# ZwwWayne/mmMOT

Measured on AMD Instinct MI355X. Metric: frame-pairs/sec (fusion+affinity fwd) at N_det=64; affinity L∞ vs CPU ref, higher is better.
Workload: dtype f16x3

## Files before the change

### include/mmmot_hip.h

```cpp
#ifndef MMMOT_HIP_H
#define MMMOT_HIP_H

#include <stddef.h>
#include <stdint.h>

#ifdef __cplusplus
extern "C" {
#endif

#define MMMOT_OK 0
#define MMMOT_EINVAL (-1)

#define MMMOT_ACT_NONE 0
#define MMMOT_ACT_RELU 1
#define MMMOT_ACT_SIGMOID 2

#define MMMOT_A_PLAIN 0
#define MMMOT_A_NORM_RELU 1
#define MMMOT_A_PAIR 2

#define MMMOT_PAIR_MULTIPLY 0
#define MMMOT_PAIR_MINUS_ABS 1
#define MMMOT_PAIR_MINUS 2

// ... 7 lines not shown

#define MMMOT_FUSION_A 0
#define MMMOT_FUSION_B 1
#define MMMOT_FUSION_C 2

int mmmot_abi_version(void);
int mmmot_device_info(int device, int* cu_count, char* arch, int arch_len);

int mmmot_conv3x3_bn_relu(const float* in, const float* wp, const float* bias,
                          float* out, int L, int H, int W, int Cin, int Cout,
                          int first, int pool, void* stream);

int mmmot_conv3x3_bn_relu_hl16_patch(const void* in, const void* wp, const float* bias, void* out,
                                     int L, int H, int W, int Cin, int Cout, int pool, const float* oscale,
                                     void* stream);
int mmmot_conv1_fused_hl16(const float* crops, const void* w1, const float* bias1, float oscale1,
                           const void* w2, const float* bias2, const float* oscale2, void* out, int L, int H, int W,
                           void* stream);
int mmmot_conv1_fused_u8(const unsigned char* crops_u8, float mean0, float mean1, float mean2, float std0, float std1,
                         float std2, const void* w1, const float* bias1, float oscale1, const void* w2,
                         const float* bias2, const float* oscale2, void* out, int L, int H, int W, int q8, void* stream);
int mmmot_conv3x3_bn_relu_hq8(const void* in, const void* wp, const float* bias, void* out,
                              int L, int H, int W, int Cin, int Cout, int pool, const float* oscale, void* stream);
int mmmot_conv1_fused_hq8(const float* crops, const void* w1, const float* bias1, float oscale1,
                          const void* w2, const float* bias2, const float* oscale2, void* out, int L, int H, int W,
                          void* stream);
int mmmot_hq8_pack(const float* x, void* y, long n, void* stream);
int mmmot_hq8_unpack(const void* x, float* y, long n, void* stream);
int mmmot_trunk_range_read(unsigned int* out4, int reset);
int mmmot_trunk_range_bind(unsigned int* counters4);
// ... 278 lines not shown
```

### mmmot_amd/_lib.py

```python
import ctypes
import os
import subprocess
import threading

_HERE = os.path.dirname(os.path.abspath(__file__))
CSRC = os.path.join(_HERE, 'csrc')
LIB_PATH = os.environ.get('MMMOT_LIB_PATH', os.path.join(_HERE, 'libmmmot_hip.so'))
SOURCES = ['conv3x3.hip', 'hl16_format.hip', 'conv3x3_hl16_patch.hip', 'gemm_rows.hip', 'gemm_wide.hip',
           'gemm_ares.hip', 'gemm_wres.hip', 'gemm_wreg.hip', 'pn_mlp64.hip', 'gram.hip', 'points_gather.hip', 'crop_resize.hip', 'crop_augment.hip','small_kernels.hip', 'backward.hip', 'train.hip', 'train_vgg.hip', 'gemm_tn_f16.hip',
           'assign.hip', 'assign_chain.hip', 'track_ids.hip', 'clear_mot.hip', 'align_points.hip', 'labels.hip', 'adam_step.hip', 'dropout.hip']
HIPCC = os.environ.get('HIPCC', '/opt/rocm/bin/hipcc')
HIPFLAGS = ['--offload-arch=gfx950', '-O3', '-std=c++17', '-fPIC']

_lock = threading.Lock()
_lib = None

c_f = ctypes.c_void_p
c_i = ctypes.c_int


class GemmArgs(ctypes.Structure):
    _fields_ = [
        ('X', c_f), ('ldx', c_i),
        ('W', c_f),
# ... 47 lines not shown
    'mmmot_abi_version': [],
    'mmmot_device_info': [c_i, ctypes.POINTER(c_i), ctypes.c_char_p, c_i],
    'mmmot_conv3x3_bn_relu': [c_f, c_f, c_f, c_f, c_i, c_i, c_i, c_i, c_i, c_i, c_i, c_f],
    'mmmot_gemm_rows': [ctypes.POINTER(GemmArgs), c_f],
    'mmmot_set_gemm_rows_variant': [c_i],
    'mmmot_gemm_ares': [ctypes.POINTER(GemmAresArgs), c_f],
    'mmmot_set_gemm_ares_variant': [c_i],
    'mmmot_gram_rows': [c_f, c_i, c_i, c_f, c_f, c_i, c_f, c_f, c_f, c_i, c_f, c_f, c_f],
    'mmmot_set_gram128_variant': [c_i],
    'mmmot_gn_finalize_gram': [c_f, c_f, c_f, c_f, c_f, c_i, c_i, c_f, c_f, c_i, c_f, c_f, ctypes.c_float, c_f, c_f, c_f, c_f],
    'mmmot_gn_finalize_gram_dbias': [c_f, c_f, c_f, c_f, c_f, c_i, c_f, c_f, c_i, c_f, c_f, c_i, c_i, c_f, c_f, ctypes.c_float,
                                     c_f, c_f, c_f, c_f],
    'mmmot_gn_finalize': [c_f, c_f, c_f, c_f, c_f, c_i, c_i, c_i, c_i, c_f, c_f, ctypes.c_float, c_f, c_f, c_f],
    'mmmot_segment_mean': [c_f, c_i, c_i, c_f, c_f, c_f, c_f, c_f, c_i, c_f, c_f, c_i, c_i, c_f, c_i, c_i, c_f],
    'mmmot_conv3x3_bn_relu_hl16_patch': [c_f, c_f, c_f, c_f, c_i, c_i, c_i, c_i, c_i, c_i, c_f, c_f],
    'mmmot_conv1_fused_hl16': [c_f, c_f, c_f, ctypes.c_float, c_f, c_f, c_f, c_f, c_i, c_i, c_i, c_f],
    'mmmot_conv3x3_bn_relu_hq8': [c_f, c_f, c_f, c_f, c_i, c_i, c_i, c_i, c_i, c_i, c_f, c_f],
    'mmmot_conv1_fused_u8': [c_f, ctypes.c_float, ctypes.c_float, ctypes.c_float, ctypes.c_float, ctypes.c_float,
                             ctypes.c_float, c_f, c_f, ctypes.c_float, c_f, c_f, c_f, c_f, c_i, c_i, c_i, c_i, c_f],
    'mmmot_u8_normalize': [c_f, c_i, c_i, c_f, c_f, c_f],
    'mmmot_conv1_fused_hq8': [c_f, c_f, c_f, ctypes.c_float, c_f, c_f, c_f, c_f, c_i, c_i, c_i, c_f],
    'mmmot_conv3x3_first_hl16': [c_f, c_f, c_f, c_f, c_i, c_i, c_i, c_i, c_f],
    'mmmot_set_patch_grid_limit': [c_i],
    'mmmot_set_patch_min_block': [c_i],
    'mmmot_trunk_range_read': [ctypes.POINTER(ctypes.c_uint), c_i],
    'mmmot_trunk_range_bind': [c_f],
    'mmmot_hl16_pack': [c_f, c_f, ctypes.c_long, c_f],
    'mmmot_hl16_unpack': [c_f, c_f, ctypes.c_long, c_f],
    'mmmot_hl16_pack_pow2': [c_f, c_f, ctypes.c_long, c_f, c_i, c_f],
    'mmmot_pow2_oscale': [c_f, c_i, c_f, c_i, c_f, c_i, c_f],
# ... 136 lines not shown
```

### mmmot_amd/csrc/conv3x3_hl16_patch.hip

```cpp
#include <atomic>
#include <type_traits>

#include "common.h"

#include "patch_common.h"

template <int BN, int BS, bool POOL, bool FUSE1 = false, bool Q8 = false, bool RAW = false PT_TIMED_TPARAM>
__global__ __launch_bounds__(512) void conv3x3_hl16_patch_kernel(
    const u32x4* __restrict__ in, const u32x4* __restrict__ wp, const float* __restrict__ bias,
    u32x4* __restrict__ out, int L, int H, int W, int Cin, int Cout, int nby, int nbx, int nblk, int ntm, int ntn,
    const float* __restrict__ oscv, Fuse1Args fz, unsigned int* __restrict__ rng) {
#include "patch_setup.inc"
  for (int item = blockIdx.x >> 3; item < clen; item += gridDim.x >> 3) {
#include "patch_loaders.inc"
#include "patch_fragments.inc"
#include "patch_prologue.inc"
#include "patch_kloop.inc"
#include "patch_epilogue.inc"
  }
}


static thread_local unsigned int* g_range_bound = nullptr;
extern "C" int mmmot_trunk_range_bind(unsigned int* counters4) {
  if (counters4 && (((uintptr_t)counters4) & 3u)) return MMMOT_EINVAL;
  g_range_bound = counters4;
// ... 44 lines not shown
  if (H <= 4 && W <= 4 && g_patch_min_block.load() != 8) return 4;
  return 8;
}

static bool pt_use_bn64(int L, int H, int W, int Cout) {
  if (Cout % 128 != 0) return true;
  const int n_cu = pt_num_cu();
  if (n_cu <= 0) return false;
  const int bs = pt_block_edge(H, W), nb = 256 / (bs * bs);
  const long nblk = (long)L * ((H + bs - 1) / bs) * ((W + bs - 1) / bs);
  const long i128 = ((nblk + nb - 1) / nb) * (Cout / 128), i64 = 2 * i128;
  auto eff = [&](long items) { return (double)items / (double)(((items + n_cu - 1) / n_cu) * n_cu); };
  return 0.85 * eff(i64) > eff(i128);
}

template <int BN, int BS, bool POOL, bool FUSE1 = false, bool Q8 = false, bool RAW = false PT_TIMED_TPARAM>
static int launch_patch_e(const void* in, const void* wp, const float* bias, void* out, int L, int H, int W, int Cin,
                        int Cout, const float* oscale, hipStream_t s, Fuse1Args fz = Fuse1Args{nullptr, nullptr, nullptr, 1.f, nullptr, {0.f, 0.f, 0.f}, {1.f, 1.f, 1.f}}) {
  const int nby = (H + BS - 1) / BS, nbx = (W + BS - 1) / BS;
  const int nblk = L * nby * nbx;
  constexpr int NB = PatchGeom<BS>::NB;
  const int ntm = (nblk + NB - 1) / NB;
  const int ntn = Cout / BN;
  const int n_cu = pt_num_cu();
  if (n_cu <= 0) return MMMOT_EINVAL;
  const int nitems = ntm * ntn;
  int grid = (n_cu / 8) * 8;
  const int glimit = g_patch_grid_limit.load();
  if (glimit > 0 && grid > glimit) grid = glimit;
  if (grid > ((nitems + 7) / 8) * 8) grid = ((nitems + 7) / 8) * 8;
  unsigned int* rng = pt_range_block();
  if (!rng) return MMMOT_EINVAL;
  hipLaunchKernelGGL((conv3x3_hl16_patch_kernel<BN, BS, POOL, FUSE1, Q8, RAW PT_TIMED_TARG(TIMED)>), dim3(grid), dim3(512), 0, s,
                     (const u32x4*)in, (const u32x4*)wp, bias, (u32x4*)out, L, H, W, Cin, Cout, nby, nbx, nblk, ntm, ntn,
                     oscale, fz, rng);
  return mm_check(hipGetLastError());
}

template <int BN, int BS, bool POOL>
static int launch_patch(const void* in, const void* wp, const float* bias, void* out, int L, int H, int W, int Cin,
                        int Cout, const float* oscale, hipStream_t s) {
#ifdef MMMOT_DEBUG
  if constexpr (BN == 128 && BS == 16)
    if (g_patch_timed) return launch_patch_e<BN, BS, POOL, false, false, false, true>(in, wp, bias, out, L, H, W, Cin, Cout, oscale, s);
#endif
  return launch_patch_e<BN, BS, POOL>(in, wp, bias, out, L, H, W, Cin, Cout, oscale, s);
}

template <int BN, int BS>
static int launch_patch_p(int pool, const void* in, const void* wp, const float* bias, void* out, int L, int H, int W,
                          int Cin, int Cout, const float* oscale, hipStream_t s) {
  return pool ? launch_patch<BN, BS, true>(in, wp, bias, out, L, H, W, Cin, Cout, oscale, s)
              : launch_patch<BN, BS, false>(in, wp, bias, out, L, H, W, Cin, Cout, oscale, s);
}

extern "C" int mmmot_conv3x3_bn_relu_hl16_patch(const void* in, const void* wp, const float* bias, void* out, int L,
                                                int H, int W, int Cin, int Cout, int pool, const float* oscale,
                                                void* stream) {
  hipStream_t s = (hipStream_t)stream;
  if (!in || !wp || !bias || !out || !oscale || L <= 0 || H <= 0 || W <= 0) return MMMOT_EINVAL;
  if (Cin % 32 != 0 || Cout % 64 != 0) return MMMOT_EINVAL;
  if (!mm_al16(in) || !mm_al16(wp) || !mm_al16(out)) return MMMOT_EINVAL;
  if ((long)L * H * W * (Cin / 4) >= (1L << 31) - 64) return MMMOT_EINVAL;
  const int bs = pt_block_edge(H, W);
  if (!pt_use_bn64(L, H, W, Cout))
    return bs == 16 ? launch_patch_p<128, 16>(pool, in, wp, bias, out, L, H, W, Cin, Cout, oscale, s)
           : bs == 8 ? launch_patch_p<128, 8>(pool, in, wp, bias, out, L, H, W, Cin, Cout, oscale, s)
                     : launch_patch_p<128, 4>(pool, in, wp, bias, out, L, H, W, Cin, Cout, oscale, s);
  return bs == 16 ? launch_patch_p<64, 16>(pool, in, wp, bias, out, L, H, W, Cin, Cout, oscale, s)
         : bs == 8 ? launch_patch_p<64, 8>(pool, in, wp, bias, out, L, H, W, Cin, Cout, oscale, s)
                   : launch_patch_p<64, 4>(pool, in, wp, bias, out, L, H, W, Cin, Cout, oscale, s);
}

extern "C" int mmmot_conv3x3_raw_hl16(const void* in, const void* wp, const float* bias, float* out, int L, int H, int W,
                                      int Cin, int Cout, const float* oscale, void* stream) {
  hipStream_t s = (hipStream_t)stream;
  if (!in || !wp || !bias || !out || !oscale || L <= 0 || H <= 0 || W <= 0) return MMMOT_EINVAL;
  if (Cin % 32 != 0 || Cout % 64 != 0) return MMMOT_EINVAL;
  if (!mm_al16(in) || !mm_al16(wp) || !mm_al16(out)) return MMMOT_EINVAL;
  if ((long)L * H * W * (Cin / 4) >= (1L << 31) - 64) return MMMOT_EINVAL;
  const int bs = pt_block_edge(H, W);
#define PT_RAW(BNV, BSV) launch_patch_e<BNV, BSV, false, false, false, true>(in, wp, bias, out, L, H, W, Cin, Cout, oscale, s)
  if (!pt_use_bn64(L, H, W, Cout)) return bs == 16 ? PT_RAW(128, 16) : bs == 8 ? PT_RAW(128, 8) : PT_RAW(128, 4);
  return bs == 16 ? PT_RAW(64, 16) : bs == 8 ? PT_RAW(64, 8) : PT_RAW(64, 4);
#undef PT_RAW
}

extern "C" int mmmot_conv1_fused_hl16(const float* crops, const void* w1, const float* bias1, float oscale1,
                                      const void* w2, const float* bias2, const float* oscale2, void* out, int L, int H,
                                      int W, void* stream) {
  hipStream_t s = (hipStream_t)stream;
  if (!crops || !w1 || !bias1 || !w2 || !bias2 || !oscale2 || !out || L <= 0 || H <= 0 || W <= 0) return MMMOT_EINVAL;
  if ((H & 1) || (W & 1) || !mm_al16(w1) || !mm_al16(w2) || !mm_al16(out)) return MMMOT_EINVAL;
  Fuse1Args fz{crops, (const u32x4*)w1, bias1, oscale1, nullptr, {0.f, 0.f, 0.f}, {1.f, 1.f, 1.f}};
#ifdef MMMOT_DEBUG
  if (g_patch_timed) return launch_patch_e<64, 16, true, true, false, false, true>(nullptr, w2, bias2, out, L, H, W, 64, 64, oscale2, s, fz);
#endif
  return launch_patch_e<64, 16, true, true>(nullptr, w2, bias2, out, L, H, W, 64, 64, oscale2, s, fz);
}

extern "C" int mmmot_conv1_fused_u8(const unsigned char* crops_u8, float mean0, float mean1, float mean2, float std0,
                                    float std1, float std2, const void* w1, const float* bias1, float oscale1,
                                    const void* w2, const float* bias2, const float* oscale2, void* out, int L, int H,
                                    int W, int q8, void* stream) {
  hipStream_t s = (hipStream_t)stream;
  if (!crops_u8 || !w1 || !bias1 || !w2 || !bias2 || !oscale2 || !out || L <= 0 || H <= 0 || W <= 0) return MMMOT_EINVAL;
  if ((H & 1) || (W & 1) || !mm_al16(w1) || !mm_al16(w2) || !mm_al16(out)) return MMMOT_EINVAL;
  if (!(std0 != 0.f) || !(std1 != 0.f) || !(std2 != 0.f)) return MMMOT_EINVAL;
  Fuse1Args fz{nullptr, (const u32x4*)w1, bias1, oscale1, crops_u8, {mean0, mean1, mean2}, {std0, std1, std2}};
  if (q8) return launch_patch_e<64, 16, true, true, true>(nullptr, w2, bias2, out, L, H, W, 64, 64, oscale2, s, fz);
  return launch_patch_e<64, 16, true, true>(nullptr, w2, bias2, out, L, H, W, 64, 64, oscale2, s, fz);
}

template <int BN, int BS>
static int launch_q8_p(int pool, const void* in, const void* wp, const float* bias, void* out, int L, int H, int W,
                       int Cin, int Cout, const float* oscale, hipStream_t s) {
#ifdef MMMOT_DEBUG
  if constexpr (BN == 128 && BS == 16)
    if (!pool && g_patch_timed) return launch_patch_e<BN, BS, false, false, true, false, true>(in, wp, bias, out, L, H, W, Cin, Cout, oscale, s);
#endif
  return pool ? launch_patch_e<BN, BS, true, false, true>(in, wp, bias, out, L, H, W, Cin, Cout, oscale, s)
              : launch_patch_e<BN, BS, false, false, true>(in, wp, bias, out, L, H, W, Cin, Cout, oscale, s);
}

extern "C" int mmmot_conv3x3_bn_relu_hq8(const void* in, const void* wp, const float* bias, void* out, int L, int H,
                                         int W, int Cin, int Cout, int pool, const float* oscale, void* stream) {
  hipStream_t s = (hipStream_t)stream;
  if (!in || !wp || !bias || !out || !oscale || L <= 0 || H <= 0 || W <= 0) return MMMOT_EINVAL;
  if (Cin % 32 != 0 || Cout % 64 != 0) return MMMOT_EINVAL;
  if (!mm_al16(in) || !mm_al16(wp) || !mm_al16(out)) return MMMOT_EINVAL;
  if ((long)L * H * W * (Cin / 4) >= (1L << 31) - 64) return MMMOT_EINVAL;
  const int bs = pt_block_edge(H, W);
  if (!pt_use_bn64(L, H, W, Cout))
    return bs == 16 ? launch_q8_p<128, 16>(pool, in, wp, bias, out, L, H, W, Cin, Cout, oscale, s)
// ... 69 lines not shown
```

### mmmot_amd/csrc/patch_epilogue.inc

```
  if constexpr (FUSE1 && !OVL) {
    raw_ready = has_next;
    if (raw_ready) fetch_raw(mt_next);
  }
  constexpr int UN = BN / 8;
  constexpr int RSTEP = 512 / UN;
  const int eu = tid % UN, er0 = tid / UN;
  const f32x8 bv = *reinterpret_cast<const f32x8*>(&bias[n0 + eu * 8]);
  const f32x8 sv = *reinterpret_cast<const f32x8*>(&oscv[n0 + eu * 8]);
  constexpr int UN16 = BN / 16;
  constexpr int RSTEP16 = 512 / UN16;
  const int eu16 = tid % UN16, er16 = tid / UN16;
  float bq[16], sq[16];
  if constexpr (Q8) {
#pragma unroll
    for (int e = 0; e < 16; ++e) {
      bq[e] = bias[n0 + eu16 * 16 + e];
      sq[e] = oscv[n0 + eu16 * 16 + e];
    }
  }
  int bcrop[G::NTB], bgy0[G::NTB], bgx0[G::NTB];
#pragma unroll
  for (int k = 0; k < G::NTB; ++k) {
    const int b = mt * G::NB + k;
    const int crop = b / nbpc;
// ... 109 lines not shown
            o[6 + hf] = l8;
          }
        }
      }
    }
  } else if constexpr (POOL) {
    const int Hq = H >> 1, Wq = W >> 1;
    constexpr int NQ = RCH;
    constexpr int NIT = (NQ + RSTEP - 1) / RSTEP;
    f32x4 va[NIT], vb[NIT];
#pragma unroll
    for (int i = 0; i < NIT; ++i) {
      const int qdl = er0 + i * RSTEP;
      mm_lds_read32(mm_lds_addr(&Cs[(qdl < NQ ? qdl : 0) * CLD + eu * 8]), va[i], vb[i]);
    }
    mm_lds_wait();
    __builtin_amdgcn_sched_barrier(0);
#pragma unroll
    for (int i = 0; i < NIT; ++i) {
      const int qdl = er0 + i * RSTEP;
      const int qd = ch * NQ + qdl;
      if (qdl >= NQ) continue;
      int blk, y, x;
      pt_row_to_pixel<BS>(qd >> 3, (qd & 7) * 4, blk, y, x);
      PT_BLK_PIXEL(blk, y, x)
      if (crop >= 0 && gy < H && gx < W && (gy >> 1) < Hq && (gx >> 1) < Wq) {
        f32x8 v = {va[i][0], va[i][1], va[i][2], va[i][3], vb[i][0], vb[i][1], vb[i][2], vb[i][3]};
#pragma unroll
        for (int e = 0; e < 8; ++e) v[e] = fmaxf(fmaf(v[e], sv[e], bv[e]), 0.f);
        {
          float vg[8];
#pragma unroll
          for (int e = 0; e < 8; ++e) vg[e] = v[e];
          pt_range_guard<8>(vg, false, rng);
        }
        u32x4 hi, lo;
        pt_split8(v, hi, lo);
        const long pix = ((long)crop * Hq + (gy >> 1)) * Wq + (gx >> 1);
        u32x4* o = out + (pix * cout8 + (n0 >> 3) + eu) * 2;
        o[0] = hi;
        o[1] = lo;
      }
    }
  } else {
    constexpr int NIT = RCH / RSTEP;
    f32x4 va[NIT], vb[NIT];
#pragma unroll
    for (int i = 0; i < NIT; ++i) mm_lds_read32(mm_lds_addr(&Cs[(er0 + i * RSTEP) * CLD + eu * 8]), va[i], vb[i]);
    mm_lds_wait();
    __builtin_amdgcn_sched_barrier(0);
#pragma unroll
    for (int i = 0; i < NIT; ++i) {
      const int rl = er0 + i * RSTEP;
      const int r = ch * RCH + rl;
      int blk, y, x;
      pt_row_to_pixel<BS>(r >> 5, r & 31, blk, y, x);
// ... 53 lines not shown
```

### mmmot_amd/csrc/patch_setup.inc

```
  static_assert(!FUSE1 || (BN == 64 && BS == 16), "the fused first layer exists for 64-channel 16x16 tiles");
  static_assert(!RAW || (!POOL && !FUSE1 && !Q8), "raw fp32 output: plain unpooled f16x3 layers");
  using G = PatchGeom<BS>;
  constexpr int WN = (BN == 128) ? 2 : 1;
  constexpr int WM = 8 / WN;
  constexpr int TM = P_BM / (WM * 32);
  constexpr int TN = BN / (WN * 32);
  constexpr int B_BYTES = BN * P_ROWB;
  constexpr int NBL = BN / 64;
  constexpr int CLD = BN + 4;
  constexpr int P0_OFF = 0;
  constexpr int P1_OFF = G::BYTES;
  constexpr int RING0 = 2 * G::BYTES;
  constexpr int LOOP_BYTES = RING0 + 3 * B_BYTES;
  constexpr int RAW_OFF = LOOP_BYTES;
  constexpr int RAW_BYTES = FUSE1 ? 3 * 20 * 20 * 4 + 64 : 0;
  constexpr bool OVL = FUSE1 && !Q8;
  constexpr int SROWS = POOL ? P_BM / 4 : P_BM;
  constexpr int NCH = (FUSE1 || POOL) ? 1 : (SROWS / 2 * CLD * 4 <= G::BYTES) ? 2 : 4;
  constexpr int RCH = SROWS / NCH;
  static_assert((FUSE1 && !OVL) ? (SROWS * CLD * 4 <= LOOP_BYTES) : (RCH * CLD * 4 <= G::BYTES), "epilogue staging does not fit");
  constexpr bool STREAM = !FUSE1 && (G::NB == 1 || G::WHOLE);
  constexpr int P2_OFF = (LOOP_BYTES + RAW_BYTES + 255) / 256 * 256;
  constexpr int POFF_OFF = OVL ? P2_OFF + G::BYTES : LOOP_BYTES + RAW_BYTES;
  constexpr int W1_OFF = POFF_OFF;
  constexpr int ZOFF = POFF_OFF + (STREAM ? G::PA * 512 * 4 : 0) + (FUSE1 ? 8192 : 0);
  static_assert(ZOFF % 256 == 0, "zero page: one aligned bank row");
  constexpr int SMEM = ZOFF + (G::WHOLE ? 256 : 0);
  static_assert(SMEM <= 160 * 1024, "LDS budget");
  __shared__ __attribute__((aligned(1024))) unsigned char smem[SMEM];

  const int tid = threadIdx.x;
  const int lane = tid & 63;
  const int wave = __builtin_amdgcn_readfirstlane(tid >> 6);
  if constexpr (G::WHOLE) {
    if (tid < 16) reinterpret_cast<u32x4*>(smem + ZOFF)[tid] = u32x4{0u, 0u, 0u, 0u};
  }

  int roff[8];
  f16x8 w1h[4], w1l[4];
  if constexpr (FUSE1) {
    const int kg1 = (threadIdx.x & 63) >> 4;
    {
// ... 154 lines not shown
```

### mmmot_amd/engine.py

```python
import contextlib
import itertools
import os
import threading

import numpy as np
import torch

from .ops import (ACT_NONE, ACT_RELU, ACT_SIGMOID, A_NORM_RELU, A_PAIR, A_PLAIN, FUSION_MODES, PAIR_OPS,
                  SOFTMAX_MODES)
from .range_guard import RangeGuard
from .tape import norm_layer

POOL_INPUT = {'f32': 0, 'hl16': 1, 'hq8': 2}
EPS = 1e-5
_SERIALS = itertools.count(1)


def check_crop_side(S):
    if S < 32 or S % 2 != 0:
        raise ValueError('crop side %d is not supported: the HIP VGG trunk needs an even side >= 32; resize the crops '
                         '(mmmot_amd.crops.crop_resize_normalize)' % S)


def check_crop_layout(dets):
# ... 24 lines not shown
        self.range_events = []
        self.last_out_of_range_forward = None
        self.out_of_range_window = None
        self._busy = threading.Lock()
        self._last_stream = None
        self._head_start = None
        ql = os.environ.get('MMMOT_Q8_LAYERS', '4,5,6,7,8,9,10,11,12')
        self.q8_layers = None if ql == 'all' else set(int(v) for v in ql.split(',') if v)
        self.pn_fused = os.environ.get('MMMOT_PN_FUSED', '1') != '0'
        self.pn_gram = os.environ.get('MMMOT_PN_GRAM', '1') != '0'
        self.pn_mlp64 = os.environ.get('MMMOT_PN_MLP64', '1') != '0'
        self.two_streams = os.environ.get('MMMOT_TWO_STREAMS', '0') == '1'
        self.pn_beside_trunk = os.environ.get('MMMOT_PN_BESIDE_TRUNK', '1') != '0'
        self._side = {}
        self.sp_fused = os.environ.get('MMMOT_SP_FUSED', '1') != '0'
        self.fuse_conv1 = os.environ.get('MMMOT_FUSE_CONV1', '1') != '0'
        self.q8_min_crop = int(os.environ.get('MMMOT_Q8_MIN_CROP', '64'))
        self.mlp = 'f32' if trunk == 'f32' else 'f16x3'
        if affinity_op not in PAIR_OPS:
            raise ValueError('unknown affinity_op %r' % (affinity_op,))
        if softmax_mode not in SOFTMAX_MODES and softmax_mode != 'none':
            softmax_mode = 'none'
        self.end_mode = end_mode
        self.P = packed
        self.ops = ops
        self.fusion = fusion
        self.affinity_op = affinity_op
        self.softmax_mode = softmax_mode
        self.neg_threshold = float(neg_threshold)
        self.score_arch = score_arch
# ... 94 lines not shown
        fmt = 'raw'
        for li, cv in enumerate(vgg):
            if fuse1 and li == 0:
                continue
            lq8 = q8 and (self.q8_layers is None or li in self.q8_layers)
            want = 'hq8' if lq8 else 'hl16'
            if f16 and fmt in ('hl16', 'hq8') and fmt != want:
                n = Lt * H * W * cv['cin']
                tmp = self.buf('vgg_recode32', n)
                (ops.hq8_unpack if fmt == 'hq8' else ops.hl16_unpack)(x, tmp)
                x = self.buf('vgg_recode', n)
                (ops.hq8_pack if want == 'hq8' else ops.hl16_pack)(tmp, x)
                fmt = want
            Ho, Wo = (H // 2, W // 2) if cv['pool'] else (H, W)
            out = self.buf('vgg%d' % (li & 1), Lt * Ho * Wo, cv['cout'])
            if self.conv_events is not None:
                e0, e1 = torch.cuda.Event(enable_timing=True), torch.cuda.Event(enable_timing=True)
                e0.record()
            if fuse1 and li == 1:
                c0 = vgg[0]
                if u8:
                    from .crops import MEAN, STD
                    ops.conv1_fused_u8(x, MEAN, STD, c0['wp16'], c0['bias'], c0['oscale'], cv['wpq8'] if lq8 else cv['wp16'],
                                       cv['bias'], cv['oscale'], out, Lt, H, W, q8=lq8)
                elif lq8:
                    ops.conv1_fused_hq8(x, c0['wp16'], c0['bias'], c0['oscale'], cv['wpq8'], cv['bias'], cv['oscale'],
                                        out, Lt, H, W)
                else:
                    ops.conv1_fused_hl16(x, c0['wp16'], c0['bias'], c0['oscale'], cv['wp16'], cv['bias'],
                                         cv['oscale'], out, Lt, H, W)
# ... 1 lines not shown
            elif f16 and li == 0:
                nq8 = q8 and (self.q8_layers is None or 1 in self.q8_layers)
                if nq8:
                    tmp = self.buf('vgg_first32', Lt * H * W, cv['cout'])
                    ops.conv3x3(x, cv['wp'], cv['bias'], tmp, Lt, H, W, cv['cin'], cv['cout'], True, cv['pool'])
                    ops.hq8_pack(tmp, out)
                else:
                    ops.conv3x3_first_hl16(x, cv['wp'], cv['bias'], out, Lt, H, W, cv['cout'])
                fmt = 'hq8' if nq8 else 'hl16'
            elif lq8:
                ops.conv3x3_hq8(x, cv['wpq8'], cv['bias'], out, Lt, H, W, cv['cin'], cv['cout'], cv['pool'], cv['oscale'])
                fmt = 'hq8'
            elif not f16:
                ops.conv3x3(x, cv['wp'], cv['bias'], out, Lt, H, W, cv['cin'], cv['cout'], li == 0, cv['pool'])
                fmt = 'f32'
            else:
                ops.conv3x3_hl16_patch(x, cv['wp16'], cv['bias'], out, Lt, H, W, cv['cin'], cv['cout'], cv['pool'],
                                       cv['oscale'])
                fmt = 'hl16'
            if self.conv_events is not None:
                e1.record()
                self.conv_events.append((li, Lt * H * W, cv['cin'], cv['cout'], e0, e1))
            x, H, W = out, Ho, Wo
            if cv['last']:
                self._stash('vgg_stage%d' % cv['stage'], x)
                self._skippool(plan, cv['stage'], x, H * W, cv['cout'], cat, fmt)

    def _mean_std(self, dev):
        key = ('mean_std', str(dev))
        if key not in self.ws:
            from .crops import MEAN, STD
            self.ws[key] = torch.tensor(list(MEAN) + list(STD), dtype=torch.float32, device=dev)
        return self.ws[key]

    def q8_in_force(self, S):
        return self.trunk == 'f16q8' and S >= self.q8_min_crop

    def trunk_elements(self, plan):
        n, H = 0, plan.S
        for cv in self.P['vgg']:
            if cv['pool']:
                H //= 2
            n += plan.Lt * H * H * cv['cout']
        return n

    def _skippool(self, plan, s, x, hw, C, cat, fmt='f32'):
        hl16 = POOL_INPUT[fmt]
        ops, Lt, hd, T = self.ops, plan.Lt, self.P['skippool'][s], plan.det_tiles
        pooled = self.buf('sp_pool', Lt, C)
        first, second, npart = plan.crop_segments(hw)
        if second is None:
            ops.segment_mean(x, C, first, pooled, use_group=False, hl16=hl16)
        else:
            partial = self.buf('sp_partial', npart, C)
            ops.segment_mean(x, C, first, partial, use_group=False, hl16=hl16)
            ops.segment_mean(partial, C, second, pooled, use_group=False)
        if self.sp_fused and hasattr(ops, 'skippool_head'):
            ops.skippool_head(pooled, C, hd, EPS, cat[:, 128 * s:128 * (s + 1)], Lt)
            return
        ln0 = self.buf('sp_ln0', Lt, C)
        ops.row_layernorm(pooled, C, hd['g0'], hd['b0'], EPS, False, ln0, Lt)
        C4 = hd['w1'].shape[0]
        h1 = self.buf('sp_h1', Lt, C4)
        self._gemm(hd, 'w1', T, C4, C, X=ln0, bias=hd['c1'], Y=h1)
        ln1 = self.buf('sp_ln1', Lt, C4)
        ops.row_layernorm(h1, C4, hd['g2'], hd['b2'], EPS, True, ln1, Lt)
# ... 319 lines not shown
```

### mmmot_amd/ops.py

```python
import contextlib
import ctypes
import os
import threading

import torch

from . import _lib

ACT_NONE, ACT_RELU, ACT_SIGMOID = 0, 1, 2
A_PLAIN, A_NORM_RELU, A_PAIR = 0, 1, 2
PAIR_OPS = {'multiply': 0, 'minus_abs': 1, 'minus': 2}
SOFTMAX_MODES = {'single': 1, 'dual': 2, 'dual_add': 3, 'dual_max': 4}
FUSION_MODES = {'A': 0, 'B': 1, 'C': 2}
LOSS_KINDS = {'bce': 0, 'l2': 1, 'l1': 2}


def _ptr(t, dtype=torch.float32):
    if t is None:
        return None
    if not t.is_cuda:
        raise RuntimeError('mmmot_amd HIP ops need device tensors (got %s); there is no CPU fallback' % t.device)
    if t.dtype != dtype:
        raise TypeError('expected %s, got %s' % (dtype, t.dtype))
    return t.data_ptr()
# ... 71 lines not shown
        try:
            with torch.cuda.stream(stream):
                yield
        finally:
            self._pinned_stream = prev

    def conv3x3(self, inp, wp, bias, out, L, H, W, Cin, Cout, first, pool):
        st = self.lib.mmmot_conv3x3_bn_relu(_ptr(inp), _ptr(wp), _ptr(bias), _ptr(out), L, H, W, Cin, Cout,
                                            int(first), int(pool), self._stream())
        _lib.check(st, 'mmmot_conv3x3_bn_relu')

    def conv3x3_hl16_patch(self, inp, wp, bias, out, L, H, W, Cin, Cout, pool, oscale):
        st = self.lib.mmmot_conv3x3_bn_relu_hl16_patch(_ptr(inp), _ptr(wp), _ptr(bias), _ptr(out), L, H, W, Cin,
                                                       Cout, int(pool), _ptr(self._osv(oscale, Cout, out)), self._stream())
        _lib.check(st, 'mmmot_conv3x3_bn_relu_hl16_patch')

    def conv1_fused_hl16(self, crops, w1, bias1, oscale1, w2, bias2, oscale2, out, L, H, W):
        st = self.lib.mmmot_conv1_fused_hl16(_ptr(crops), _ptr(w1), _ptr(bias1), float(oscale1), _ptr(w2),
                                             _ptr(bias2), _ptr(self._osv(oscale2, 64, out)), _ptr(out), L, H, W, self._stream())
        _lib.check(st, 'mmmot_conv1_fused_hl16')

    def conv3x3_hq8(self, inp, wp, bias, out, L, H, W, Cin, Cout, pool, oscale):
        st = self.lib.mmmot_conv3x3_bn_relu_hq8(_ptr(inp), _ptr(wp), _ptr(bias), _ptr(out), L, H, W, Cin, Cout,
                                                int(pool), _ptr(self._osv(oscale, Cout, out)), self._stream())
        _lib.check(st, 'mmmot_conv3x3_bn_relu_hq8')

    def conv1_fused_hq8(self, crops, w1, bias1, oscale1, w2, bias2, oscale2, out, L, H, W):
        st = self.lib.mmmot_conv1_fused_hq8(_ptr(crops), _ptr(w1), _ptr(bias1), float(oscale1), _ptr(w2),
                                            _ptr(bias2), _ptr(self._osv(oscale2, 64, out)), _ptr(out), L, H, W, self._stream())
        _lib.check(st, 'mmmot_conv1_fused_hq8')
# ... 411 lines not shown
```

### mmmot_amd/plan.py

```python
import collections

import numpy as np
import torch

TILE = 128


class TableUpload:

    def __init__(self, device):
        self.device = device
        self.items = []

    def add(self, obj, attr, arr):
        self.items.append((obj, attr, np.ascontiguousarray(arr, dtype=np.int32).reshape(-1)))

    def flush(self):
        if not self.items:
            return
        offs, total = [], 0
        for _, _, a in self.items:
            offs.append(total)
            total += (a.size + 3) // 4 * 4
        buf = np.zeros(max(total, 4), np.int32)
# ... 181 lines not shown
                r0 = int(self.pair_tiles.h_g_row0[g])
                v_cnt.append(M)
                for j in range(M):
                    s_start.append(r0 + j); s_count.append(N); s_stride.append(M); s_group.append(g)
                    omap.append(0 * nR * Lt + ri * Lt + b0 + j)
                v_cnt.append(N)
                for i in range(N):
                    s_start.append(r0 + i * M); s_count.append(M); s_stride.append(1); s_group.append(g)
                    omap.append(1 * nR * Lt + ri * Lt + a0 + i)
        self.v_tiles = RowTiles(v_cnt, device)
        self.v_segs = Segments(s_start, s_count, s_stride, s_group, device)
        up(omap, 'v_omap')
        if use_images and self.S >= 32:
            for sh in (4, 8, 16, 32):
                self._crop_segments((self.S // sh) ** 2, device)
        up_all.flush()

    def _crop_segments(self, hw, device):
        Lt = self.Lt
        S = -(-hw // 256)
        if S <= 1:
            self.crop_segs[hw] = (Segments(np.arange(Lt) * hw, np.full(Lt, hw), np.ones(Lt), np.zeros(Lt), device), None, 0)
            return self.crop_segs[hw]
        chunk = 256
        l, c = np.repeat(np.arange(Lt), S), np.tile(np.arange(S), Lt)
        start = l * hw + c * chunk
        count = np.minimum(chunk, hw - c * chunk)
        first = Segments(start, count, np.ones(Lt * S), np.zeros(Lt * S), device, div=np.ones(Lt * S))
        second = Segments(np.arange(Lt) * S, np.full(Lt, S), np.ones(Lt), np.zeros(Lt), device, div=np.full(Lt, hw))
        self.crop_segs[hw] = (first, second, Lt * S)
        return self.crop_segs[hw]

    def crop_segments(self, hw):
        if hw not in self.crop_segs:
            self._crop_segments(hw, self.device)
        return self.crop_segs[hw]

    def tail_crops(self):
        if self.B != 1 or len(self.frame_counts[0]) != 2:
            raise ValueError('appearance rows of the leading frame need a plan of one frame pair (B = 1, two frames)')
        cp = self.__dict__.get('_tail_crops')
        if cp is None:
            cp = self._tail_crops = CropPlan(self.frame_counts[0][1], self.S, self.device)
        return cp


class CropPlan:

    def __init__(self, L, S, device):
        self.device = device
        self.Lt, self.S = int(L), int(S)
        if self.Lt < 1:
            raise ValueError('a crop plan needs >= 1 crop')
        up = TableUpload(device)
        self.det_tiles = RowTiles([self.Lt], up)
        self.crop_segs = {}
        if self.S >= 32:
            for sh in (4, 8, 16, 32):
                self._crop_segments((self.S // sh) ** 2, up)
        up.flush()

    _crop_segments = BatchPlan._crop_segments
    crop_segments = BatchPlan.crop_segments


class PlanCache:

    def __init__(self, capacity):
        self.capacity = max(int(capacity), 1)
        self._plans = collections.OrderedDict()

    def get(self, key, build):
        plan = self._plans.get(key)
        if plan is not None:
            self._plans.move_to_end(key)
            return plan
        while len(self._plans) >= self.capacity:
            self._plans.popitem(last=False)
# ... 9 lines not shown
```

### mmmot_amd/profiler.py

```python
import time

import torch

PEAK_F16X3_TFLOPS = 2500.0 / 3.0
PEAK_F32_TFLOPS = 157.3
PEAK_HBM_TBS = 8.0


def _rows(t):
    return int(getattr(t, 'R', 0))


def _seg_rows(segs):
    return int(segs.h_count.sum())


def _conv(name):
    def cost(a, k):
        inp, wp, bias, out, L, H, W, Cin, Cout = a[:9]
        pool = a[10] if name == 'conv3x3' else a[9]
        Ho, Wo = (H // 2, W // 2) if pool else (H, W)
        fl = 2.0 * L * H * W * 9 * Cin * Cout
        by = 4.0 * (L * H * W * Cin + L * Ho * Wo * Cout + 9 * Cin * Cout)
        return ('trunk conv %d->%d @%dx%d%s' % (Cin, Cout, H, W, ' +pool' if pool else ''), fl, by)
    return cost


def _conv1_fused(a, k):
    i = max(j for j, v in enumerate(a) if torch.is_tensor(v))
    L, H, W = a[i + 1:i + 4]
    fl = 2.0 * L * H * W * 9 * (3 * 64 + 64 * 64)
    by = (1.0 if a[0].dtype == torch.uint8 else 4.0) * L * H * W * 3 + 4.0 * L * (H // 2) * (W // 2) * 64
    return ('trunk conv1_1+conv1_2 (fused) 3->64->64 @%dx%d +pool' % (H, W), fl, by)


def _gemm(a, k):
    W, tiles, N, K = a[:4]
    R = _rows(tiles)
    amode = k.get('amode', 0)
    kind = {0: 'plain', 1: 'norm+relu prologue', 2: 'pair prologue'}[amode]
    by = 4.0 * N * K + (4.0 * R * N if k.get('Y') is not None else 0.0)
    if amode != 2 and k.get('X') is not None:
# ... 39 lines not shown

def _latency(label):
    return lambda a, k: (label, 0.0, 0.0)


def _layer1(a, k):
    X, W, bias, Y, part, tiles = a[:6]
    R = _rows(tiles)
    Kin = int(W.shape[1])
    return ('PointNet layer %d->64 (points in)' % Kin, 2.0 * R * Kin * 64, 4.0 * R * (Kin + 64))


COSTS = {
    'conv3x3': _conv('conv3x3'),
    'conv3x3_hl16_patch': _conv('hl16'),
    'conv3x3_hq8': _conv('hq8'),
    'conv1_fused_hl16': _conv1_fused,
    'conv1_fused_hq8': _conv1_fused,
    'conv1_fused_u8': _conv1_fused,
    'conv3x3_first_hl16': lambda a, k: ('trunk conv1_1 3->%d (fp32 MFMA)' % a[7], 2.0 * a[4] * a[5] * a[6] * 27 * a[7],
                                        4.0 * a[4] * a[5] * a[6] * (3 + a[7])),
    'gemm': _gemm,
    'gemm_ares': _gemm_ares,
    'pn_mlp64': _pn_mlp64,
    'gram_rows': _gram,
    'gn_finalize_gram': _latency('GroupNorm scale/shift from the Gram matrix'),
    'gn_finalize_gram_dbias': _latency('GroupNorm scale/shift from the Gram matrix'),
    'gn_finalize': _latency('GroupNorm scale/shift from tile partials'),
    'segment_mean': _segment_mean,
    'rowdot': _rowdot,
# ... 103 lines not shown
```

Before: 287.3.

## Emit per-block pooled channel sums from last conv of each stage for skip-pool

Adds a PSUM variant of the pooled hl16 patch conv kernel. The epilogue reduces the pooled outputs per spatial block via shuffles (and LDS when needed) and writes per-block channel partial sums. The skip-pool then runs segment_mean over these few block sums instead of re-reading the whole stage output, removing a full re-read of the activation. In exchange it adds reduction work, LDS use and a barrier to the conv epilogue, plus an fp32 partial buffer.

After: 287.4 (median of 2 runs). Within noise of the previous version (+0.0%).

```diff
diff --git a/include/mmmot_hip.h b/include/mmmot_hip.h
--- a/include/mmmot_hip.h
+++ b/include/mmmot_hip.h
@@ -45,6 +45,10 @@
 int mmmot_conv3x3_bn_relu_hl16_patch(const void* in, const void* wp, const float* bias, void* out,
                                      int L, int H, int W, int Cin, int Cout, int pool, const float* oscale,
                                      void* stream);
+int mmmot_conv3x3_bn_relu_hl16_patch_pool(const void* in, const void* wp, const float* bias, void* out,
+                                          int L, int H, int W, int Cin, int Cout, const float* oscale,
+                                          float* pool_part, void* stream);
+int mmmot_patch_pool_blocks(int L, int H, int W);
 int mmmot_conv1_fused_hl16(const float* crops, const void* w1, const float* bias1, float oscale1,
                            const void* w2, const float* bias2, const float* oscale2, void* out, int L, int H, int W,
                            void* stream);
diff --git a/mmmot_amd/_lib.py b/mmmot_amd/_lib.py
--- a/mmmot_amd/_lib.py
+++ b/mmmot_amd/_lib.py
@@ -85,6 +85,8 @@
     'mmmot_gn_finalize': [c_f, c_f, c_f, c_f, c_f, c_i, c_i, c_i, c_i, c_f, c_f, ctypes.c_float, c_f, c_f, c_f],
     'mmmot_segment_mean': [c_f, c_i, c_i, c_f, c_f, c_f, c_f, c_f, c_i, c_f, c_f, c_i, c_i, c_f, c_i, c_i, c_f],
     'mmmot_conv3x3_bn_relu_hl16_patch': [c_f, c_f, c_f, c_f, c_i, c_i, c_i, c_i, c_i, c_i, c_f, c_f],
+    'mmmot_conv3x3_bn_relu_hl16_patch_pool': [c_f, c_f, c_f, c_f, c_i, c_i, c_i, c_i, c_i, c_f, c_f, c_f],
+    'mmmot_patch_pool_blocks': [c_i, c_i, c_i],
     'mmmot_conv1_fused_hl16': [c_f, c_f, c_f, ctypes.c_float, c_f, c_f, c_f, c_f, c_i, c_i, c_i, c_f],
     'mmmot_conv3x3_bn_relu_hq8': [c_f, c_f, c_f, c_f, c_i, c_i, c_i, c_i, c_i, c_i, c_f, c_f],
     'mmmot_conv1_fused_u8': [c_f, ctypes.c_float, ctypes.c_float, ctypes.c_float, ctypes.c_float, ctypes.c_float,
diff --git a/mmmot_amd/csrc/conv3x3_hl16_patch.hip b/mmmot_amd/csrc/conv3x3_hl16_patch.hip
--- a/mmmot_amd/csrc/conv3x3_hl16_patch.hip
+++ b/mmmot_amd/csrc/conv3x3_hl16_patch.hip
@@ -5,11 +5,11 @@
 
 #include "patch_common.h"
 
-template <int BN, int BS, bool POOL, bool FUSE1 = false, bool Q8 = false, bool RAW = false PT_TIMED_TPARAM>
+template <int BN, int BS, bool POOL, bool FUSE1 = false, bool Q8 = false, bool RAW = false, bool PSUM = false PT_TIMED_TPARAM>
 __global__ __launch_bounds__(512) void conv3x3_hl16_patch_kernel(
     const u32x4* __restrict__ in, const u32x4* __restrict__ wp, const float* __restrict__ bias,
     u32x4* __restrict__ out, int L, int H, int W, int Cin, int Cout, int nby, int nbx, int nblk, int ntm, int ntn,
-    const float* __restrict__ oscv, Fuse1Args fz, unsigned int* __restrict__ rng) {
+    const float* __restrict__ oscv, Fuse1Args fz, unsigned int* __restrict__ rng, float* __restrict__ pool_part) {
 #include "patch_setup.inc"
   for (int item = blockIdx.x >> 3; item < clen; item += gridDim.x >> 3) {
 #include "patch_loaders.inc"
@@ -84,9 +84,10 @@
   return 0.85 * eff(i64) > eff(i128);
 }
 
-template <int BN, int BS, bool POOL, bool FUSE1 = false, bool Q8 = false, bool RAW = false PT_TIMED_TPARAM>
+template <int BN, int BS, bool POOL, bool FUSE1 = false, bool Q8 = false, bool RAW = false, bool PSUM = false PT_TIMED_TPARAM>
 static int launch_patch_e(const void* in, const void* wp, const float* bias, void* out, int L, int H, int W, int Cin,
-                        int Cout, const float* oscale, hipStream_t s, Fuse1Args fz = Fuse1Args{nullptr, nullptr, nullptr, 1.f, nullptr, {0.f, 0.f, 0.f}, {1.f, 1.f, 1.f}}) {
+                        int Cout, const float* oscale, hipStream_t s, Fuse1Args fz = Fuse1Args{nullptr, nullptr, nullptr, 1.f, nullptr, {0.f, 0.f, 0.f}, {1.f, 1.f, 1.f}},
+                        float* pool_part = nullptr) {
   const int nby = (H + BS - 1) / BS, nbx = (W + BS - 1) / BS;
   const int nblk = L * nby * nbx;
   constexpr int NB = PatchGeom<BS>::NB;
@@ -101,9 +102,9 @@
   if (grid > ((nitems + 7) / 8) * 8) grid = ((nitems + 7) / 8) * 8;
   unsigned int* rng = pt_range_block();
   if (!rng) return MMMOT_EINVAL;
-  hipLaunchKernelGGL((conv3x3_hl16_patch_kernel<BN, BS, POOL, FUSE1, Q8, RAW PT_TIMED_TARG(TIMED)>), dim3(grid), dim3(512), 0, s,
+  hipLaunchKernelGGL((conv3x3_hl16_patch_kernel<BN, BS, POOL, FUSE1, Q8, RAW, PSUM PT_TIMED_TARG(TIMED)>), dim3(grid), dim3(512), 0, s,
                      (const u32x4*)in, (const u32x4*)wp, bias, (u32x4*)out, L, H, W, Cin, Cout, nby, nbx, nblk, ntm, ntn,
-                     oscale, fz, rng);
+                     oscale, fz, rng, pool_part);
   return mm_check(hipGetLastError());
 }
 
@@ -112,7 +113,7 @@
                         int Cout, const float* oscale, hipStream_t s) {
 #ifdef MMMOT_DEBUG
   if constexpr (BN == 128 && BS == 16)
-    if (g_patch_timed) return launch_patch_e<BN, BS, POOL, false, false, false, true>(in, wp, bias, out, L, H, W, Cin, Cout, oscale, s);
+    if (g_patch_timed) return launch_patch_e<BN, BS, POOL, false, false, false, false, true>(in, wp, bias, out, L, H, W, Cin, Cout, oscale, s);
 #endif
   return launch_patch_e<BN, BS, POOL>(in, wp, bias, out, L, H, W, Cin, Cout, oscale, s);
 }
@@ -142,6 +143,30 @@
                    : launch_patch_p<64, 4>(pool, in, wp, bias, out, L, H, W, Cin, Cout, oscale, s);
 }
 
+extern "C" int mmmot_patch_pool_blocks(int L, int H, int W) {
+  if (L <= 0 || H <= 0 || W <= 0) return MMMOT_EINVAL;
+  const int bs = pt_block_edge(H, W);
+  const long n = (long)L * ((H + bs - 1) / bs) * ((W + bs - 1) / bs);
+  return n < (1L << 31) ? (int)n : MMMOT_EINVAL;
+}
+
+extern "C" int mmmot_conv3x3_bn_relu_hl16_patch_pool(const void* in, const void* wp, const float* bias, void* out, int L,
+                                                     int H, int W, int Cin, int Cout, const float* oscale,
+                                                     float* pool_part, void* stream) {
+  hipStream_t s = (hipStream_t)stream;
+  if (!in || !wp || !bias || !out || !oscale || !pool_part || L <= 0 || H <= 0 || W <= 0) return MMMOT_EINVAL;
+  if (Cin % 32 != 0 || Cout % 64 != 0) return MMMOT_EINVAL;
+  if (!mm_al16(in) || !mm_al16(wp) || !mm_al16(out) || !mm_al16(pool_part)) return MMMOT_EINVAL;
+  if ((long)L * H * W * (Cin / 4) >= (1L << 31) - 64) return MMMOT_EINVAL;
+  const int bs = pt_block_edge(H, W);
+  const Fuse1Args nofz{nullptr, nullptr, nullptr, 1.f, nullptr, {0.f, 0.f, 0.f}, {1.f, 1.f, 1.f}};
+#define PT_PSUM(BNV, BSV) \
+  launch_patch_e<BNV, BSV, true, false, false, false, true>(in, wp, bias, out, L, H, W, Cin, Cout, oscale, s, nofz, pool_part)
+  if (!pt_use_bn64(L, H, W, Cout)) return bs == 16 ? PT_PSUM(128, 16) : bs == 8 ? PT_PSUM(128, 8) : PT_PSUM(128, 4);
+  return bs == 16 ? PT_PSUM(64, 16) : bs == 8 ? PT_PSUM(64, 8) : PT_PSUM(64, 4);
+#undef PT_PSUM
+}
+
 extern "C" int mmmot_conv3x3_raw_hl16(const void* in, const void* wp, const float* bias, float* out, int L, int H, int W,
                                       int Cin, int Cout, const float* oscale, void* stream) {
   hipStream_t s = (hipStream_t)stream;
@@ -164,7 +189,7 @@
   if ((H & 1) || (W & 1) || !mm_al16(w1) || !mm_al16(w2) || !mm_al16(out)) return MMMOT_EINVAL;
   Fuse1Args fz{crops, (const u32x4*)w1, bias1, oscale1, nullptr, {0.f, 0.f, 0.f}, {1.f, 1.f, 1.f}};
 #ifdef MMMOT_DEBUG
-  if (g_patch_timed) return launch_patch_e<64, 16, true, true, false, false, true>(nullptr, w2, bias2, out, L, H, W, 64, 64, oscale2, s, fz);
+  if (g_patch_timed) return launch_patch_e<64, 16, true, true, false, false, false, true>(nullptr, w2, bias2, out, L, H, W, 64, 64, oscale2, s, fz);
 #endif
   return launch_patch_e<64, 16, true, true>(nullptr, w2, bias2, out, L, H, W, 64, 64, oscale2, s, fz);
 }
@@ -187,7 +212,7 @@
                        int Cin, int Cout, const float* oscale, hipStream_t s) {
 #ifdef MMMOT_DEBUG
   if constexpr (BN == 128 && BS == 16)
-    if (!pool && g_patch_timed) return launch_patch_e<BN, BS, false, false, true, false, true>(in, wp, bias, out, L, H, W, Cin, Cout, oscale, s);
+    if (!pool && g_patch_timed) return launch_patch_e<BN, BS, false, false, true, false, false, true>(in, wp, bias, out, L, H, W, Cin, Cout, oscale, s);
 #endif
   return pool ? launch_patch_e<BN, BS, true, false, true>(in, wp, bias, out, L, H, W, Cin, Cout, oscale, s)
               : launch_patch_e<BN, BS, false, false, true>(in, wp, bias, out, L, H, W, Cin, Cout, oscale, s);
diff --git a/mmmot_amd/csrc/patch_epilogue.inc b/mmmot_amd/csrc/patch_epilogue.inc
--- a/mmmot_amd/csrc/patch_epilogue.inc
+++ b/mmmot_amd/csrc/patch_epilogue.inc
@@ -147,6 +147,13 @@
       const int qdl = er0 + i * RSTEP;
       mm_lds_read32(mm_lds_addr(&Cs[(qdl < NQ ? qdl : 0) * CLD + eu * 8]), va[i], vb[i]);
     }
+    float ps[PSUM ? NIT : 1][8];
+    if constexpr (PSUM) {
+#pragma unroll
+      for (int i = 0; i < NIT; ++i)
+#pragma unroll
+        for (int e = 0; e < 8; ++e) ps[i][e] = 0.f;
+    }
     mm_lds_wait();
     __builtin_amdgcn_sched_barrier(0);
 #pragma unroll
@@ -173,6 +180,77 @@
         u32x4* o = out + (pix * cout8 + (n0 >> 3) + eu) * 2;
         o[0] = hi;
         o[1] = lo;
+        if constexpr (PSUM) {
+#pragma unroll
+          for (int k = 0; k < 4; ++k) {
+            const unsigned hw = hi[k], lw = lo[k];
+            const f16x2 h2 = __builtin_bit_cast(f16x2, hw), l2 = __builtin_bit_cast(f16x2, lw);
+            ps[i][2 * k] = mm_hl_join(h2[0], l2[0]);
+            ps[i][2 * k + 1] = mm_hl_join(h2[1], l2[1]);
+          }
+        }
+      }
+    }
+    if constexpr (PSUM) {
+      constexpr int RPW = 64 / UN;
+      constexpr int QPB = 64 / G::NB;
+      constexpr int RG = RPW < QPB ? RPW : QPB;
+      constexpr int GPB = QPB / RG;
+      static_assert(NIT * RSTEP == 64 && RSTEP == 8 * RPW, "pool partials: rows of a tile");
+#pragma unroll
+      for (int j = 0; j < NIT; ++j)
+#pragma unroll
+        for (int e = 0; e < 8; ++e) {
+          float x = ps[j][e];
+#pragma unroll
+          for (int o = UN; o < UN * RG; o <<= 1) x = (o == 32) ? mm_xor32_sum(x) : x + __shfl_xor(x, o);
+          ps[j][e] = x;
+        }
+      if constexpr (GPB == 1) {
+        if (lane % (UN * RG) < UN) {
+#pragma unroll
+          for (int j = 0; j < NIT; ++j) {
+            const int b = mt * G::NB + (wave * RPW + j * RSTEP) / QPB + lane / (UN * RG);
+            if (b < nblk) {
+              f32x4* o = reinterpret_cast<f32x4*>(pool_part + (long)b * Cout + n0 + eu * 8);
+              o[0] = f32x4{ps[j][0], ps[j][1], ps[j][2], ps[j][3]};
+              o[1] = f32x4{ps[j][4], ps[j][5], ps[j][6], ps[j][7]};
+            }
+          }
+        }
+      } else {
+        static_assert(NIT * 8 * BN * 4 <= PSUM_BYTES && NIT * 8 == G::NB * GPB, "pool partials: LDS area");
+        float* Ps = reinterpret_cast<float*>(smem + PSUM_OFF);
+        if (lane < UN) {
+#pragma unroll
+          for (int j = 0; j < NIT; ++j) {
+            f32x4* d = reinterpret_cast<f32x4*>(&Ps[(j * 8 + wave) * BN + eu * 8]);
+            d[0] = f32x4{ps[j][0], ps[j][1], ps[j][2], ps[j][3]};
+            d[1] = f32x4{ps[j][4], ps[j][5], ps[j][6], ps[j][7]};
+          }
+        }
+        mm_lds_barrier();
+        if (tid < G::NB * UN) {
+          const int kb = tid / UN;
+          f32x4 qa[GPB], qb[GPB];
+#pragma unroll
+          for (int g = 0; g < GPB; ++g) mm_lds_read32(mm_lds_addr(&Ps[(kb * GPB + g) * BN + eu * 8]), qa[g], qb[g]);
+          mm_lds_wait();
+          __builtin_amdgcn_sched_barrier(0);
+#pragma unroll
+          for (int st = 1; st < GPB; st <<= 1)
+#pragma unroll
+            for (int g = 0; g < GPB; g += 2 * st) {
+              qa[g] += qa[g + st];
+              qb[g] += qb[g + st];
+            }
+          const int b = mt * G::NB + kb;
+          if (b < nblk) {
+            f32x4* o = reinterpret_cast<f32x4*>(pool_part + (long)b * Cout + n0 + eu * 8);
+            o[0] = qa[0];
+            o[1] = qb[0];
+          }
+        }
       }
     }
   } else {
diff --git a/mmmot_amd/csrc/patch_setup.inc b/mmmot_amd/csrc/patch_setup.inc
--- a/mmmot_amd/csrc/patch_setup.inc
+++ b/mmmot_amd/csrc/patch_setup.inc
@@ -1,5 +1,6 @@
   static_assert(!FUSE1 || (BN == 64 && BS == 16), "the fused first layer exists for 64-channel 16x16 tiles");
   static_assert(!RAW || (!POOL && !FUSE1 && !Q8), "raw fp32 output: plain unpooled f16x3 layers");
+  static_assert(!PSUM || (POOL && !FUSE1 && !Q8), "pool partials: pooled f16x3 inference layers");
   using G = PatchGeom<BS>;
   constexpr int WN = (BN == 128) ? 2 : 1;
   constexpr int WM = 8 / WN;
@@ -25,7 +26,9 @@
   constexpr int W1_OFF = POFF_OFF;
   constexpr int ZOFF = POFF_OFF + (STREAM ? G::PA * 512 * 4 : 0) + (FUSE1 ? 8192 : 0);
   static_assert(ZOFF % 256 == 0, "zero page: one aligned bank row");
-  constexpr int SMEM = ZOFF + (G::WHOLE ? 256 : 0);
+  constexpr int PSUM_OFF = ZOFF + (G::WHOLE ? 256 : 0);
+  constexpr int PSUM_BYTES = (PSUM && !G::WHOLE) ? (BN / 64) * 8 * BN * 4 : 0;
+  constexpr int SMEM = PSUM_OFF + PSUM_BYTES;
   static_assert(SMEM <= 160 * 1024, "LDS budget");
   __shared__ __attribute__((aligned(1024))) unsigned char smem[SMEM];
 
diff --git a/mmmot_amd/engine.py b/mmmot_amd/engine.py
--- a/mmmot_amd/engine.py
+++ b/mmmot_amd/engine.py
@@ -62,6 +62,7 @@
         self.pn_beside_trunk = os.environ.get('MMMOT_PN_BESIDE_TRUNK', '1') != '0'
         self._side = {}
         self.sp_fused = os.environ.get('MMMOT_SP_FUSED', '1') != '0'
+        self.pool_in_producer = os.environ.get('MMMOT_POOL_IN_PRODUCER', '1') != '0'
         self.fuse_conv1 = os.environ.get('MMMOT_FUSE_CONV1', '1') != '0'
         self.q8_min_crop = int(os.environ.get('MMMOT_Q8_MIN_CROP', '64'))
         self.mlp = 'f32' if trunk == 'f32' else 'f16x3'
@@ -186,6 +187,7 @@
                 fmt = want
             Ho, Wo = (H // 2, W // 2) if cv['pool'] else (H, W)
             out = self.buf('vgg%d' % (li & 1), Lt * Ho * Wo, cv['cout'])
+            pool_part = None
             if self.conv_events is not None:
                 e0, e1 = torch.cuda.Event(enable_timing=True), torch.cuda.Event(enable_timing=True)
                 e0.record()
@@ -217,6 +219,13 @@
             elif not f16:
                 ops.conv3x3(x, cv['wp'], cv['bias'], out, Lt, H, W, cv['cin'], cv['cout'], li == 0, cv['pool'])
                 fmt = 'f32'
+            elif cv['pool'] and cv['last'] and self.pool_in_producer and hasattr(ops, 'conv3x3_hl16_patch_pool'):
+                nblk = ops.patch_pool_blocks(Lt, H, W)
+                blocks = self.buf('sp_blocks', nblk, cv['cout'])
+                ops.conv3x3_hl16_patch_pool(x, cv['wp16'], cv['bias'], out, Lt, H, W, cv['cin'], cv['cout'], cv['oscale'],
+                                            blocks)
+                pool_part = (blocks, nblk // Lt)
+                fmt = 'hl16'
             else:
                 ops.conv3x3_hl16_patch(x, cv['wp16'], cv['bias'], out, Lt, H, W, cv['cin'], cv['cout'], cv['pool'],
                                        cv['oscale'])
@@ -227,7 +236,7 @@
             x, H, W = out, Ho, Wo
             if cv['last']:
                 self._stash('vgg_stage%d' % cv['stage'], x)
-                self._skippool(plan, cv['stage'], x, H * W, cv['cout'], cat, fmt)
+                self._skippool(plan, cv['stage'], x, H * W, cv['cout'], cat, fmt, pool_part)
 
     def _mean_std(self, dev):
         key = ('mean_std', str(dev))
@@ -247,12 +256,15 @@
             n += plan.Lt * H * H * cv['cout']
         return n
 
-    def _skippool(self, plan, s, x, hw, C, cat, fmt='f32'):
+    def _skippool(self, plan, s, x, hw, C, cat, fmt='f32', pool_part=None):
         hl16 = POOL_INPUT[fmt]
         ops, Lt, hd, T = self.ops, plan.Lt, self.P['skippool'][s], plan.det_tiles
         pooled = self.buf('sp_pool', Lt, C)
         first, second, npart = plan.crop_segments(hw)
-        if second is None:
+        if pool_part is not None:
+            blocks, nbpc = pool_part
+            ops.segment_mean(blocks, C, plan.pool_block_segments(nbpc, hw), pooled, use_group=False)
+        elif second is None:
             ops.segment_mean(x, C, first, pooled, use_group=False, hl16=hl16)
         else:
             partial = self.buf('sp_partial', npart, C)
diff --git a/mmmot_amd/ops.py b/mmmot_amd/ops.py
--- a/mmmot_amd/ops.py
+++ b/mmmot_amd/ops.py
@@ -109,6 +109,18 @@
         st = self.lib.mmmot_conv3x3_bn_relu_hl16_patch(_ptr(inp), _ptr(wp), _ptr(bias), _ptr(out), L, H, W, Cin,
                                                        Cout, int(pool), _ptr(self._osv(oscale, Cout, out)), self._stream())
         _lib.check(st, 'mmmot_conv3x3_bn_relu_hl16_patch')
+
+    def conv3x3_hl16_patch_pool(self, inp, wp, bias, out, L, H, W, Cin, Cout, oscale, pool_part):
+        st = self.lib.mmmot_conv3x3_bn_relu_hl16_patch_pool(_ptr(inp), _ptr(wp), _ptr(bias), _ptr(out), L, H, W, Cin, Cout,
+                                                            _ptr(self._osv(oscale, Cout, out)), _ptr(pool_part),
+                                                            self._stream())
+        _lib.check(st, 'mmmot_conv3x3_bn_relu_hl16_patch_pool')
+
+    def patch_pool_blocks(self, L, H, W):
+        n = self.lib.mmmot_patch_pool_blocks(L, H, W)
+        if n <= 0:
+            _lib.check(-1, 'mmmot_patch_pool_blocks')
+        return n
 
     def conv1_fused_hl16(self, crops, w1, bias1, oscale1, w2, bias2, oscale2, out, L, H, W):
         st = self.lib.mmmot_conv1_fused_hl16(_ptr(crops), _ptr(w1), _ptr(bias1), float(oscale1), _ptr(w2),
diff --git a/mmmot_amd/plan.py b/mmmot_amd/plan.py
--- a/mmmot_amd/plan.py
+++ b/mmmot_amd/plan.py
@@ -219,6 +219,9 @@
         if use_images and self.S >= 32:
             for sh in (4, 8, 16, 32):
                 self._crop_segments((self.S // sh) ** 2, device)
+            self._pool_block_segments_of_trunk(device)
+        else:
+            self.pool_segs = {}
         up_all.flush()
 
     def _crop_segments(self, hw, device):
@@ -241,6 +244,24 @@
             self._crop_segments(hw, self.device)
         return self.crop_segs[hw]
 
+    def _pool_block_segments(self, nbpc, hw, device):
+        Lt = self.Lt
+        self.pool_segs[(nbpc, hw)] = Segments(np.arange(Lt) * nbpc, np.full(Lt, nbpc), np.ones(Lt), np.zeros(Lt), device,
+                                              div=np.full(Lt, hw))
+        return self.pool_segs[(nbpc, hw)]
+
+    def _pool_block_segments_of_trunk(self, device):
+        self.pool_segs = {}
+        H = self.S // 2
+        for _ in range(4):
+            bs = 16 if H > 8 else (4 if H <= 4 else 8)
+            self._pool_block_segments((-(-H // bs)) ** 2, (H // 2) ** 2, device)
+            H //= 2
+
+    def pool_block_segments(self, nbpc, hw):
+        segs = self.pool_segs.get((nbpc, hw))
+        return segs if segs is not None else self._pool_block_segments(nbpc, hw, self.device)
+
     def tail_crops(self):
         if self.B != 1 or len(self.frame_counts[0]) != 2:
             raise ValueError('appearance rows of the leading frame need a plan of one frame pair (B = 1, two frames)')
@@ -263,10 +284,16 @@
         if self.S >= 32:
             for sh in (4, 8, 16, 32):
                 self._crop_segments((self.S // sh) ** 2, up)
+            self._pool_block_segments_of_trunk(up)
+        else:
+            self.pool_segs = {}
         up.flush()
 
     _crop_segments = BatchPlan._crop_segments
     crop_segments = BatchPlan.crop_segments
+    _pool_block_segments = BatchPlan._pool_block_segments
+    _pool_block_segments_of_trunk = BatchPlan._pool_block_segments_of_trunk
+    pool_block_segments = BatchPlan.pool_block_segments
 
 
 class PlanCache:
diff --git a/mmmot_amd/profiler.py b/mmmot_amd/profiler.py
--- a/mmmot_amd/profiler.py
+++ b/mmmot_amd/profiler.py
@@ -26,6 +26,13 @@
     return cost
 
 
+def _conv_pool_part(a, k):
+    inp, wp, bias, out, L, H, W, Cin, Cout = a[:9]
+    fl = 2.0 * L * H * W * 9 * Cin * Cout
+    by = 4.0 * (L * H * W * Cin + L * (H // 2) * (W // 2) * Cout + 9 * Cin * Cout + a[10].numel())
+    return ('trunk conv %d->%d @%dx%d +pool +block sums' % (Cin, Cout, H, W), fl, by)
+
+
 def _conv1_fused(a, k):
     i = max(j for j, v in enumerate(a) if torch.is_tensor(v))
     L, H, W = a[i + 1:i + 4]
@@ -95,6 +102,7 @@
 COSTS = {
     'conv3x3': _conv('conv3x3'),
     'conv3x3_hl16_patch': _conv('hl16'),
+    'conv3x3_hl16_patch_pool': _conv_pool_part,
     'conv3x3_hq8': _conv('hq8'),
     'conv1_fused_hl16': _conv1_fused,
     'conv1_fused_hq8': _conv1_fused,
```
